# secondmind-labs/markovflow

Hardware: AMD Instinct MI355X
Metric: Kalman log-lik steps/sec (BxT) at d=6 (higher is better)
Workload: dtype f64; 1 GPU; KalmanFilter.log_likelihood B=1024/GPU T=10000 d=6 m=1 f64 (sum of two Matern-5/2, north-star target config); series_per_gpu=1024, state_dim=6, output_dim=1, parallelism=batch-sharded x1, one scalar RCCL all-reduce

## Files before the change

markovflow_amd/csrc/mf_head_carry.hpp:

```cpp
#pragma once

namespace mf {

template <int ROWB, int UNIT, typename Keep> struct HeadCarry {
    static constexpr int LINE = 128;
    static constexpr int MAXT = 2;
    static constexpr int UG = (ROWB + UNIT - 1) / UNIT;
    static constexpr int STEP = ROWB % LINE;
    static constexpr int cand(int t) {
        int n = 0;
        for (int u = 0; u < UG; ++u)
            if (Keep::keep(u, UNIT) && (u + 1) * UNIT <= LINE - 4) { if (n == t) return u; ++n; }
        return -1;
    }
    static constexpr int count_cand() { int n = 0; while (n < MAXT && cand(n) >= 0) ++n; return n; }
    static constexpr int tail_index(int u) { for (int t = 0; t < count_cand(); ++t) if (cand(t) == u) return t; return -1; }
    static constexpr unsigned carried_units(int r) {
        r &= LINE - 1;
        if (r == 0) return 0u;
        const int room = LINE - r;
        unsigned m = 0u;
        for (int u = 0; u < UG; ++u) {
            if (!Keep::keep(u, UNIT) || u * UNIT >= room) continue;
            const int t = tail_index(u);
            if (t < 0 || (u + 1) * UNIT > room) return 0u;
            m |= 1u << t;
        }
        return m;
    }
    static constexpr unsigned table(int t) {
        unsigned m = 0u;
        for (int g = 0; g < 32; ++g) if ((carried_units(4 * g) >> t) & 1u) m |= 1u << g;
        return m;
    }
    static constexpr unsigned TAB0 = table(0), TAB1 = table(1);
    static constexpr int period() { int p = 1, r = STEP; while (r % LINE) { r += STEP; ++p; } return p; }
    static constexpr int PERIOD = (ROWB % 4 == 0) ? period() : 0;
    static constexpr bool USABLE = ROWB % 4 == 0 && ROWB >= LINE && STEP != 0 && Keep::keep(UG - 1, UNIT) && (TAB0 | TAB1) != 0u;
    static constexpr int NT = USABLE ? count_cand() : 0;
    static constexpr int tail_unit(int t) { return cand(t); }

    static constexpr bool carried(unsigned addr, int t) { return (((t == 0 ? TAB0 : TAB1) >> ((addr & (LINE - 1)) >> 2)) & 1u) != 0u; }

    static constexpr unsigned consumer_bits(unsigned addr0) {
        unsigned m = 0u;
        for (int t = 0; t < NT; ++t)
            for (int p = 0; p < PERIOD; ++p) if (carried(addr0 + (unsigned)(p * STEP), t)) m |= 1u << (t * PERIOD + p);
        return m;
    }
    static constexpr unsigned producer_bits(unsigned addr0, int kind) {
        unsigned m = 0u;
        for (int p = 0; p < PERIOD; ++p) {
            bool f = true;
            if (kind >= 1 + MAXT) f = carried(addr0 + (unsigned)((p + 1) * STEP), kind - 1 - MAXT);
            else if (kind >= 1) f = !carried(addr0 + (unsigned)(p * STEP), kind - 1);
            if (f) m |= 1u << p;
        }
        return m;
    }
};

template <int ROWB, typename Keep, bool TAIL = false> struct Stream {
    static constexpr int UNIT = (ROWB >= 16) ? 16 : 4;
    static constexpr int UG = (ROWB + UNIT - 1) / UNIT;
    static constexpr int count_kept() { int n = 0; for (int u = 0; u < UG; ++u) n += Keep::keep(u, UNIT) ? 1 : 0; return n; }
    using HC = HeadCarry<ROWB, UNIT, Keep>;
    static constexpr int UB = count_kept();
    static constexpr int NT = TAIL ? HC::NT : 0;
    static constexpr int U = UB + NT;
    static constexpr int NI = U;
    static constexpr int LDS_BYTES = 64 * U * UNIT;
    static constexpr bool ALL = (UB == UG) && NT == 0;
    static constexpr int global_unit(int c) {
        int n = 0;
        for (int u = 0; u < UG; ++u) if (Keep::keep(u, UNIT)) { if (n == c) return u; ++n; }
        return -1;
    }
    static constexpr int global_offset(int c) { return c < UB ? global_unit(c) * UNIT : ROWB + HC::tail_unit(c - UB) * UNIT; }
    static constexpr int unit_kind(int c) {
        if (c >= UB) return 1 + HC::MAXT + (c - UB);
        for (int t = 0; t < NT; ++t) if (global_unit(c) == HC::tail_unit(t)) return 1 + t;
        return 0;
    }
    static constexpr int compact_unit(int gu) {
        int n = 0;
        for (int u = 0; u < gu; ++u) n += Keep::keep(u, UNIT) ? 1 : 0;
        return n;
    }
};

struct KeepAll { static constexpr bool keep(int, int) { return true; } };
template <int D, int S> struct KeepLower {
    static constexpr bool keep(int u, int unit) {
        const int lo = u * unit, hi = lo + unit;
        for (int i = 0; i < D; ++i) {
            const int a = (i * D) * S, b = (i * D + i + 1) * S;
            if (a < hi && lo < b) return true;
        }
        return false;
    }
};

}
```

markovflow_amd/csrc/mf_kf_lds.hpp:

```cpp
#pragma once
#include "mf_kernels.hpp"
#include "mf_head_carry.hpp"
#include <type_traits>
#ifndef MF_PUMPMASK
#define MF_PUMPMASK 63
#endif

namespace mf {

typedef int mf_v4i __attribute__((ext_vector_type(4)));

#define MF_POLICY_STR_0 ""
#define MF_POLICY_STR_1 " nt"
#define MF_POLICY_STR_2 " sc1"
#define MF_POLICY_STR_3 " sc0 sc1"
#define MF_POLICY_STR_4 " sc0"
#define MF_POLICY_CAT(n) MF_POLICY_STR_##n
#define MF_POLICY_OF(n) MF_POLICY_CAT(n)
#ifndef MF_POLW
#define MF_POLW 1
#endif
#ifndef MF_POLN
#define MF_POLN 0
#endif
#define MF_POLICY_WIDE MF_POLICY_OF(MF_POLW)
#define MF_POLICY_NARROW MF_POLICY_OF(MF_POLN)
#define MF_DMA_HEAD "s_nop 4\n\ts_mov_b32 %0, m0\n\ts_mov_b32 m0, %2\n\ts_nop 0\n\t"
#define MF_DMA_TAIL "s_mov_b32 m0, %0"
#define MF_DMA_X4(v, pol) "buffer_load_dwordx4 " v ", %1, 0 offen" pol " lds\n\t"
#define MF_DMA_X1(v, pol) "buffer_load_dword " v ", %1, 0 offen" pol " lds\n\t"
#define MF_DMA_STEP4 "s_add_u32 m0, m0, 0x400\n\ts_nop 0\n\t"
#define MF_DMA_STEP1 "s_add_u32 m0, m0, 0x100\n\ts_nop 0\n\t"
template <bool WIDE, int N> MF_DEV void dma_b128_group(mf_v4i srd, unsigned lds_addr, const unsigned* v) {
    unsigned keep;
    static_assert(N >= 1 && N <= 4, "group size");
#define MF_DMA_B128_BODY(POL)                                                                                                       \
    if constexpr (N == 1)                                                                                                           \
        asm volatile(MF_DMA_HEAD MF_DMA_X4("%3", POL) MF_DMA_TAIL : "=&s"(keep) : "s"(srd), "s"(lds_addr), "v"(v[0]) : "memory", "scc"); \
    else if constexpr (N == 2)                                                                                                      \
        asm volatile(MF_DMA_HEAD MF_DMA_X4("%3", POL) MF_DMA_STEP4 MF_DMA_X4("%4", POL) MF_DMA_TAIL                                 \
                     : "=&s"(keep) : "s"(srd), "s"(lds_addr), "v"(v[0]), "v"(v[1]) : "memory", "scc");                              \
    else if constexpr (N == 3)                                                                                                      \
        asm volatile(MF_DMA_HEAD MF_DMA_X4("%3", POL) MF_DMA_STEP4 MF_DMA_X4("%4", POL) MF_DMA_STEP4 MF_DMA_X4("%5", POL) MF_DMA_TAIL \
                     : "=&s"(keep) : "s"(srd), "s"(lds_addr), "v"(v[0]), "v"(v[1]), "v"(v[2]) : "memory", "scc");                   \
    else                                                                                                                            \
        asm volatile(MF_DMA_HEAD MF_DMA_X4("%3", POL) MF_DMA_STEP4 MF_DMA_X4("%4", POL) MF_DMA_STEP4 MF_DMA_X4("%5", POL)           \
                     MF_DMA_STEP4 MF_DMA_X4("%6", POL) MF_DMA_TAIL                                                                  \
                     : "=&s"(keep) : "s"(srd), "s"(lds_addr), "v"(v[0]), "v"(v[1]), "v"(v[2]), "v"(v[3]) : "memory", "scc");
    if (WIDE) { MF_DMA_B128_BODY(MF_POLICY_WIDE) } else { MF_DMA_B128_BODY(MF_POLICY_NARROW) }
#undef MF_DMA_B128_BODY
}
template <int N> MF_DEV void dma_b32_group(mf_v4i srd, unsigned lds_addr, const unsigned* v) {
    unsigned keep;
    static_assert(N >= 1 && N <= 4, "group size");
    if constexpr (N == 1)
        asm volatile(MF_DMA_HEAD MF_DMA_X1("%3", MF_POLICY_NARROW) MF_DMA_TAIL : "=&s"(keep) : "s"(srd), "s"(lds_addr), "v"(v[0]) : "memory", "scc");
    else if constexpr (N == 2)
        asm volatile(MF_DMA_HEAD MF_DMA_X1("%3", MF_POLICY_NARROW) MF_DMA_STEP1 MF_DMA_X1("%4", MF_POLICY_NARROW) MF_DMA_TAIL
                     : "=&s"(keep) : "s"(srd), "s"(lds_addr), "v"(v[0]), "v"(v[1]) : "memory", "scc");
    else if constexpr (N == 3)
        asm volatile(MF_DMA_HEAD MF_DMA_X1("%3", MF_POLICY_NARROW) MF_DMA_STEP1 MF_DMA_X1("%4", MF_POLICY_NARROW) MF_DMA_STEP1
                     MF_DMA_X1("%5", MF_POLICY_NARROW) MF_DMA_TAIL
                     : "=&s"(keep) : "s"(srd), "s"(lds_addr), "v"(v[0]), "v"(v[1]), "v"(v[2]) : "memory", "scc");
    else
        asm volatile(MF_DMA_HEAD MF_DMA_X1("%3", MF_POLICY_NARROW) MF_DMA_STEP1 MF_DMA_X1("%4", MF_POLICY_NARROW) MF_DMA_STEP1
                     MF_DMA_X1("%5", MF_POLICY_NARROW) MF_DMA_STEP1 MF_DMA_X1("%6", MF_POLICY_NARROW) MF_DMA_TAIL
                     : "=&s"(keep) : "s"(srd), "s"(lds_addr), "v"(v[0]), "v"(v[1]), "v"(v[2]), "v"(v[3]) : "memory", "scc");
}


constexpr unsigned MF_DMA_INVALID = 0xF0000000u;
constexpr unsigned long long MF_DMA_MAXREC = 0xE0000000ull;

template <typename St, typename = void> struct StreamTail { static constexpr int NT = 0, PERIOD = 1; };
template <typename St> struct StreamTail<St, std::enable_if_t<(St::NT > 0)>> { static constexpr int NT = St::NT, PERIOD = St::HC::PERIOD; };

template <typename St> struct DmaStream {
    using TL = StreamTail<St>;
    unsigned vo[St::NI];
    static constexpr int PB = TL::PERIOD;
    static constexpr int FW = TL::NT > 0 ? (St::NI * PB + 31) / 32 : 1;
    unsigned fm[FW];
    MF_DEV void init(const char* smem, int lane, int rel_tab, int gtab, unsigned base_lo = 0u) {
        const int q0 = lane / St::U, c0 = lane - q0 * St::U;
        if constexpr (TL::NT > 0) { MF_UNROLL for (int w = 0; w < FW; ++w) fm[w] = 0u; }
        MF_UNROLL for (int i = 0; i < St::NI; ++i) {
            const int a = (64 * i) / St::U, b = (64 * i) % St::U;
            int cu = c0 + b;
            const int carry = cu >= St::U ? 1 : 0;
            cu -= carry * St::U;
            const int row = q0 + a + carry;
            const unsigned rel = *reinterpret_cast<const unsigned*>(smem + rel_tab + row * 4);
            unsigned off;
            if (St::ALL) off = (unsigned)cu * St::UNIT;
            else off = *reinterpret_cast<const unsigned*>(smem + gtab + cu * 4);
            vo[i] = rel + off;
            if constexpr (TL::NT > 0) {
                static_assert(PB < 32 && 32 % PB == 0, "an instruction's schedule bits do not straddle two words");
                int kind = 0;
                MF_UNROLL for (int cc = 0; cc < St::U; ++cc) if (St::unit_kind(cc) != 0 && cu == cc) kind = St::unit_kind(cc);
                unsigned bits = (1u << PB) - 1u;
                MF_UNROLL for (int kk = 1; kk <= 2 * St::HC::MAXT; ++kk)
                    if (kind == kk) bits = St::HC::producer_bits(base_lo + rel, kk);
                fm[(i * PB) / 32] |= bits << ((i * PB) % 32);
            }
#ifdef MF_EXPERIMENT
            if (pack_base != 0xffffffffu && rel < MF_DMA_INVALID)
                vo[i] |= ((((pack_base + rel) >> 5) & 3u) << 29) | ((unsigned)(off / St::UNIT) << 24);
#endif
        }
    }
#ifdef MF_EXPERIMENT
    unsigned pack_base = 0xffffffffu;
    unsigned step_next = 0;
    bool skip_carried = false;
    MF_DEV unsigned exp_offset(unsigned v) const {
        if (pack_base == 0xffffffffu || v >= MF_DMA_INVALID) return v;
        const unsigned phase = ((v >> 29) + step_next) & 3u, gu = (v >> 24) & 31u, off = v & 0xffffffu;
        const bool carried = skip_carried && phase != 0u && gu < 8u - 2u * phase;
        return carried ? MF_DMA_INVALID : off;
    }
#endif
    template <int I0, int I1, bool SCHED = false> MF_DEV void issue(mf_v4i srd, unsigned lds_base, unsigned phase = 0u) const {
        constexpr int HI = I1 < St::NI ? I1 : St::NI;
        if constexpr (I0 < HI) {
            constexpr int N = (HI - I0) < 4 ? (HI - I0) : 4;
            unsigned voff[N];
            MF_UNROLL for (int k = 0; k < N; ++k) {
#ifdef MF_EXPERIMENT
                voff[k] = exp_offset(vo[I0 + k]);
#else
                voff[k] = vo[I0 + k];
#endif
                if constexpr (SCHED && TL::NT > 0)
                    voff[k] = ((fm[((I0 + k) * PB) / 32] >> (((I0 + k) * PB) % 32 + phase)) & 1u) ? voff[k] : MF_DMA_INVALID;
            }
            if (St::UNIT == 16) dma_b128_group<(St::UG >= 8), N>(srd, lds_base + I0 * 1024, voff);
            else dma_b32_group<N>(srd, lds_base + I0 * 256, voff);
            issue<I0 + N, I1, SCHED>(srd, lds_base, phase);
        }
    }
};

MF_DEV unsigned long long uniform64(unsigned long long x) {
    const unsigned lo = (unsigned)__builtin_amdgcn_readfirstlane((int)(unsigned)x);
    const unsigned hi = (unsigned)__builtin_amdgcn_readfirstlane((int)(unsigned)(x >> 32));
    return ((unsigned long long)hi << 32) | lo;
}

MF_DEV mf_v4i make_srd(unsigned long long base, unsigned long long end, int debug = 0) {
    unsigned long long rem = end > base ? end - base : 0ull;
    if (debug & 1) rem = 0;
    if (rem > MF_DMA_MAXREC) rem = MF_DMA_MAXREC;
    mf_v4i srd;
    srd.x = __builtin_amdgcn_readfirstlane((int)(unsigned)base);
    srd.y = __builtin_amdgcn_readfirstlane((int)((unsigned)(base >> 32) & 0xffffu));
    srd.z = __builtin_amdgcn_readfirstlane((int)(unsigned)rem);
    srd.w = 0x00020000;
    return srd;
}

template <typename T, typename St> struct RowReader {
    const char* row;
    MF_DEV RowReader(const char* smem, int lds_off, int lane) : row(smem + lds_off + lane * (St::U * St::UNIT)) {}
    MF_DEV T at(int e) const {
        const int byte = e * (int)sizeof(T);
        const int gu = byte / St::UNIT;
        const int off = St::compact_unit(gu) * St::UNIT + (byte - gu * St::UNIT);
        return *reinterpret_cast<const T*>(row + off);
    }
    MF_DEV T tail_at(int t, int k) const { return *reinterpret_cast<const T*>(row + (St::UB + t) * St::UNIT + k * (int)sizeof(T)); }
};

template <typename T, int D, int M, bool RSTEP = false, int BG = 1, bool CARRY = false> struct KfLdsCfg {
    static constexpr int S = sizeof(T);
    static constexpr int BGRP = BG;
    using StA = Stream<D * D * S, KeepAll>;
    using StC0 = Stream<D * D * S, KeepLower<D, S>>;
    using StCT = Stream<D * D * S, KeepLower<D, S>, true>;
    using Stb = Stream<BG * D * S, KeepAll>;
    using StH = Stream<BG * M * D * S, KeepAll>;
    static constexpr int YG = (M == 1) ? 4 : 1;
    using Sty = Stream<YG * M * S, KeepAll>;
    using StR = Stream<M * M * S, KeepAll>;
    static constexpr bool RS = RSTEP;
    static constexpr int QUARTER_CU = (160 * 1024) / 4;
    static constexpr int TABLE_BYTES = 5 * 256 + ((StCT::U * 4 + 15) / 16) * 16;
    static constexpr int IMAGE_T = StA::LDS_BYTES + StCT::LDS_BYTES + Stb::LDS_BYTES + StH::LDS_BYTES + ((Sty::LDS_BYTES + 15) / 16) * 16 +
                                   (RSTEP ? ((StR::LDS_BYTES + 15) / 16) * 16 : 0);
    static constexpr bool TAIL = CARRY && StCT::NT > 0 && !StC0::ALL && StCT::NI * StCT::HC::PERIOD <= 64 &&
                                 StCT::NT * StCT::HC::PERIOD <= 32 && IMAGE_T <= QUARTER_CU && TABLE_BYTES <= IMAGE_T &&
                                 (StA::NI + StCT::NI + Stb::NI + StH::NI + Sty::NI + (RSTEP ? StR::NI : 0)) < 64;
    using StC = Stream<D * D * S, KeepLower<D, S>, TAIL>;
    static constexpr int OFF_A = 0;
    static constexpr int OFF_C = OFF_A + StA::LDS_BYTES;
    static constexpr int OFF_b = OFF_C + StC::LDS_BYTES;
    static constexpr int OFF_H = OFF_b + Stb::LDS_BYTES;
    static constexpr int OFF_y = OFF_H + StH::LDS_BYTES;
    static constexpr int OFF_R = OFF_y + ((Sty::LDS_BYTES + 15) / 16) * 16;
    static constexpr int IMAGE_END = OFF_R + (RSTEP ? ((StR::LDS_BYTES + 15) / 16) * 16 : 0);
    static constexpr int OFF_relA = TAIL ? 0 : IMAGE_END;
    static constexpr int OFF_relb = OFF_relA + 256;
    static constexpr int OFF_relH = OFF_relb + 256;
    static constexpr int OFF_rely = OFF_relH + 256;
    static constexpr int OFF_relR = OFF_rely + 256;
    static constexpr int OFF_gtabC = OFF_relR + 256;
    static constexpr int LDS_TOTAL = TAIL ? IMAGE_END : OFF_gtabC + ((StC::U * 4 + 15) / 16) * 16;
    static constexpr bool SUPPORTED =
                                      (StA::NI + StC::NI + Stb::NI + StH::NI + Sty::NI + (RSTEP ? StR::NI : 0)) < 64 &&
                                      LDS_TOTAL <= 64 * 1024;
};

template <typename T, int D, int M, bool RSTEP = false> using KfChunkCfg = KfLdsCfg<T, D, M, RSTEP, 1, true>;
static_assert(KfChunkCfg<double, 6, 1>::TAIL && KfChunkCfg<double, 6, 1>::LDS_TOTAL <= 40960, "fp64 d = 6: four wavefronts per CU");

template <typename Cfg> struct KfPump {
    static constexpr int N_SMALL = Cfg::StC::NI + Cfg::Stb::NI + Cfg::StH::NI + Cfg::Sty::NI + (Cfg::RS ? Cfg::StR::NI : 0);
    static constexpr int N_BIG = Cfg::StA::NI;
    const DmaStream<typename Cfg::StA>& dA; const DmaStream<typename Cfg::StC>& dC;
    const DmaStream<typename Cfg::Stb>& db; const DmaStream<typename Cfg::StH>& dH;
    const DmaStream<typename Cfg::Sty>& dy; const DmaStream<typename Cfg::StR>& dR;
    mf_v4i sA, sC, sb, sH, sy, sR;
    unsigned lds0;
    bool more;
    bool yfetch = true;
    unsigned cphase = 0;
    template <int K> MF_DEV void small() const {
        if (!((MF_PUMPMASK >> K) & 1)) return;
        small_do<K>();
    }
    template <int K> MF_DEV void small_do() const {
        if (!more) return;
        constexpr int HC = (Cfg::StC::NI + 1) / 2;
        if (K == 0) dC.template issue<0, HC, true>(sC, lds0 + Cfg::OFF_C, cphase);
        else {
            dC.template issue<HC, 64, true>(sC, lds0 + Cfg::OFF_C, cphase);
            db.template issue<0, 64>(sb, lds0 + Cfg::OFF_b);
            dH.template issue<0, 64>(sH, lds0 + Cfg::OFF_H);
            if (yfetch) dy.template issue<0, 64>(sy, lds0 + Cfg::OFF_y);
            if (Cfg::RS) dR.template issue<0, 64>(sR, lds0 + Cfg::OFF_R);
        }
    }
    template <int K> MF_DEV void all() const {
        dC.template issue<0, 64>(sC, lds0 + Cfg::OFF_C);
        db.template issue<0, 64>(sb, lds0 + Cfg::OFF_b);
        dH.template issue<0, 64>(sH, lds0 + Cfg::OFF_H);
        dy.template issue<0, 64>(sy, lds0 + Cfg::OFF_y);
        if (Cfg::RS) dR.template issue<0, 64>(sR, lds0 + Cfg::OFF_R);
        dA.template issue<0, 64>(sA, lds0 + Cfg::OFF_A);
    }
    template <int K> MF_DEV void big() const {
        if (!((MF_PUMPMASK >> (K + 2)) & 1)) return;
        big_do<K>();
    }
    MF_DEV void unpumped() const {
        if (!((MF_PUMPMASK >> 0) & 1)) small_do<0>();
        if (!((MF_PUMPMASK >> 1) & 1)) small_do<1>();
        if (!((MF_PUMPMASK >> 2) & 1)) big_do<0>();
        if (!((MF_PUMPMASK >> 3) & 1)) big_do<1>();
        if (!((MF_PUMPMASK >> 4) & 1)) big_do<2>();
        if (!((MF_PUMPMASK >> 5) & 1)) big_do<3>();
    }
    template <int K> MF_DEV void big_do() const {
        if (!more) return;
        constexpr int Q = (Cfg::StA::NI + 3) / 4;
        dA.template issue<K * Q, (K + 1) * Q>(sA, lds0 + Cfg::OFF_A);
    }
};

template <typename T, int D, int M, bool SPIKE, bool FIRST, typename Pump>
MF_DEV void kf_lds_step(Elim<T, D, SPIKE>& E, LogAcc<T>& laC, T& acc_yry, T& acc_ww, const T (&C)[D][D],
                        const T (&mvec)[D], const T (&hk)[M * D], const T (&yk)[M], const T (&Rsh)[M * M],
                        T (&Bm)[D][D], const Pump& pump, bool active, bool sep_lane) {
    const bool sep = FIRST && sep_lane, ord = active && !sep;
    T Ci[D][D], w[D], btw[D];
    if (active) {
        tri_inv_lower<T, D>(C, Ci, laC, E.bad);
        laC.renorm();
    }
    pump.template small<0>();
    if (active) {
        trimul_lower_vec<T, D>(Ci, mvec, w);
        acc_ww += dot_self<T, D>(w);
    }
    pump.template small<1>();
    pump.template big<0>();
    if (active) {
        trimul_lower_inplace<T, D, D>(Ci, Bm);
        gemv_t<T, D, D>(Bm, w, btw);
    }
    pump.template big<1>();
    if (FIRST && active && sep) {
        syrk_tn_lower<T, D, D>(Bm, E.GU, T(1));
        MF_UNROLL for (int i = 0; i < D; ++i) E.gU[i] = -btw[i];
    }
    if (ord) {
        syrk_tn_lower<T, D, D>(Bm, E.Phi, T(1));
        MF_UNROLL for (int i = 0; i < D; ++i) E.t[i] -= btw[i];
    }
    pump.template big<2>();
    if (FIRST && active && sep) {
        neg_trimulT_lower_inplace<T, D, D>(Ci, Bm);
        MF_UNROLL for (int i = 0; i < D; ++i) MF_UNROLL for (int j = 0; j < D; ++j) E.X[i][j] = Bm[i][j];
    }
    if (ord) E.eliminate_main();
    pump.template big<3>();
    if (FIRST && active && sep) {
        trimulT_self_lower<T, D>(Ci, E.Phi);
        trimulT_lower_vec<T, D>(Ci, w, E.t);
        acc_yry += Obs<T, D, M>::apply(hk, yk, Rsh, M, E.Phi, E.t);
    }
    if (ord) {
        E.eliminate_spike();
        trsm_right_lower_t<T, D, D>(E.Phi, E.Li, Bm);
        neg_trimulT_lower_inplace<T, D, D>(Ci, Bm);
        T Dn[D][D], rn[D];
        trimulT_self_lower<T, D>(Ci, Dn);
        trimulT_lower_vec<T, D>(Ci, w, rn);
        acc_yry += Obs<T, D, M>::apply(hk, yk, Rsh, M, Dn, rn);
        E.advance(Bm, Dn, rn);
    }
}

template <typename T, int D, int M, bool SPIKE, bool RSTEP = false>
__global__ void __launch_bounds__(64) kf_chunk_lds_kernel(KfArgs<T> a, long L, RedSys<T> out) {
    using Cfg = KfChunkCfg<T, D, M, RSTEP>;
    extern __shared__ __attribute__((aligned(16))) char smem[];
    const int lane = threadIdx.x;
    const long total = a.B * a.P;
    const long id_raw = (long)blockIdx.x * 64 + lane;
    const bool valid = id_raw < total;
    const long id = valid ? id_raw : total - 1;
    const long s = id / a.P, c = id % a.P;
    const long nt = a.Tn - 1;
    const long tau0 = c * L;
    long len = nt - tau0;
    if (len > L) len = L;
    if (len < 0 || !valid) len = 0;
    constexpr int S = sizeof(T);

    const unsigned long long offA = (unsigned long long)(s * nt + tau0) * (D * D * S);
    const unsigned long long offb = (unsigned long long)(s * nt + tau0) * (D * S);
    const unsigned long long offH = (unsigned long long)(s * a.Tn + tau0 + 1) * (M * D * S);
    const unsigned long long offy = (unsigned long long)(s * a.Tn + tau0 + 1) * (M * S);
    const unsigned long long offR = (unsigned long long)(s * a.Tn + tau0 + 1) * (M * M * S);
    const unsigned long long offA0 = uniform64(offA), offb0 = uniform64(offb);
    const unsigned long long offH0 = uniform64(offH), offy0 = uniform64(offy), offR0 = uniform64(offR);
    const bool rowok = valid && len > 0;
    {
        unsigned* tab = reinterpret_cast<unsigned*>(smem);
        tab[Cfg::OFF_relA / 4 + lane] = rowok ? (unsigned)(offA - offA0) : MF_DMA_INVALID;
        tab[Cfg::OFF_relb / 4 + lane] = rowok ? (unsigned)(offb - offb0) : MF_DMA_INVALID;
        tab[Cfg::OFF_relH / 4 + lane] = rowok ? (unsigned)(offH - offH0) : MF_DMA_INVALID;
        tab[Cfg::OFF_rely / 4 + lane] = rowok ? (unsigned)(offy - offy0) : MF_DMA_INVALID;
        tab[Cfg::OFF_relR / 4 + lane] = rowok ? (unsigned)(offR - offR0) : MF_DMA_INVALID;
        if (lane < Cfg::StC::U) {
            unsigned g = 0;
            MF_UNROLL for (int cc = 0; cc < Cfg::StC::U; ++cc) if (lane == cc) g = (unsigned)Cfg::StC::global_offset(cc);
            tab[Cfg::OFF_gtabC / 4 + lane] = g;
        }
    }
    DmaStream<typename Cfg::StA> dA;
    DmaStream<typename Cfg::StC> dC;
    DmaStream<typename Cfg::Stb> db;
    DmaStream<typename Cfg::StH> dH;
    DmaStream<typename Cfg::Sty> dy;
    DmaStream<typename Cfg::StR> dR;
    unsigned long long pA = (unsigned long long)a.A + offA0, pC = (unsigned long long)a.cholQ + offA0;
    unsigned long long pb = (unsigned long long)a.b + offb0, pH = (unsigned long long)a.H + offH0;
    unsigned long long py = (unsigned long long)a.y + offy0;
    unsigned long long pR = (unsigned long long)a.Rinv + (RSTEP ? offR0 : 0ull);
    const unsigned long long eA = (unsigned long long)a.A + (unsigned long long)a.B * nt * (D * D * S);
    const unsigned long long eC = (unsigned long long)a.cholQ + (unsigned long long)a.B * nt * (D * D * S);
    const unsigned long long eb = (unsigned long long)a.b + (unsigned long long)a.B * nt * (D * S);
    const unsigned long long eH = (unsigned long long)a.H + (unsigned long long)a.B * a.Tn * (M * D * S);
    const unsigned long long ey = (unsigned long long)a.y + (unsigned long long)a.B * a.Tn * (M * S);
    const unsigned long long eR = (unsigned long long)a.Rinv + (RSTEP ? (unsigned long long)a.B * a.Tn * (M * M * S) : 0ull);
    const unsigned lds0 = (unsigned)(size_t)smem;

    Elim<T, D, SPIKE> E;
    E.init();
    LogAcc<T> laC;
    laC.init();
    T acc_yry = T(0), acc_ww = T(0);
    T Rsh[M * M];
    MF_UNROLL for (int i = 0; i < M * M; ++i) Rsh[i] = RSTEP ? (valid ? a.Rinv[(s * a.Tn) * M * M + i] : T(0)) : a.Rinv[i];
    if (valid && c == 0) {
        T C[D][D], Ci[D][D], mvec[D], w[D];
        load_lower<T, D>(a.cholP0 + s * D * D, C);
        load_vec<T, D>(a.mu0 + s * D, mvec);
        tri_inv_lower<T, D>(C, Ci, laC, E.bad);
        laC.renorm();
        trimul_lower_vec<T, D>(Ci, mvec, w);
        acc_ww += dot_self<T, D>(w);
        trimulT_self_lower<T, D>(Ci, E.Phi);
        trimulT_lower_vec<T, D>(Ci, w, E.t);
        acc_yry += Obs<T, D, M>::apply(a.H + (s * a.Tn) * M * D, a.y + (s * a.Tn) * M, Rsh, M, E.Phi, E.t);
    }

    long nsteps = len;
    MF_UNROLL for (int off = 32; off > 0; off >>= 1) {
        const long o = __shfl_xor((long long)nsteps, off);
        nsteps = o > nsteps ? o : nsteps;
    }
    nsteps = __builtin_amdgcn_readfirstlane((int)nsteps);
    asm volatile("s_waitcnt vmcnt(0) lgkmcnt(0)" ::: "memory");
#ifdef MF_EXPERIMENT
    if (a.debug & 8) {
        dA.pack_base = (unsigned)__builtin_amdgcn_readfirstlane((int)(unsigned)pA);
        dC.pack_base = (unsigned)__builtin_amdgcn_readfirstlane((int)(unsigned)pC);
    }
#endif
    dA.init(smem, lane, Cfg::OFF_relA, 0);
    dC.init(smem, lane, Cfg::OFF_relA, Cfg::OFF_gtabC, (unsigned)pC);
    db.init(smem, lane, Cfg::OFF_relb, 0);
    dH.init(smem, lane, Cfg::OFF_relH, 0);
    dy.init(smem, lane, Cfg::OFF_rely, 0);
    if (RSTEP) dR.init(smem, lane, Cfg::OFF_relR, 0);
    asm volatile("s_waitcnt lgkmcnt(0)" ::: "memory");
    using HC = typename Cfg::StC::HC;
    constexpr int NTAIL = Cfg::StC::NT, CPER = NTAIL > 0 ? HC::PERIOD : 1, UEL = Cfg::StC::UNIT / S;
    const unsigned cbits = NTAIL > 0 ? HC::consumer_bits((unsigned)((unsigned long long)a.cholQ + offA)) : 0u;
    T cv[NTAIL > 0 ? NTAIL : 1][UEL];
    MF_UNROLL for (int t = 0; t < (NTAIL > 0 ? NTAIL : 1); ++t) MF_UNROLL for (int k = 0; k < UEL; ++k) cv[t][k] = T(0);

    const RowReader<T, typename Cfg::StA> rA(smem, Cfg::OFF_A, lane);
    const RowReader<T, typename Cfg::StC> rC(smem, Cfg::OFF_C, lane);
    const RowReader<T, typename Cfg::Stb> rb(smem, Cfg::OFF_b, lane);
    const RowReader<T, typename Cfg::StH> rH(smem, Cfg::OFF_H, lane);
    const RowReader<T, typename Cfg::Sty> ry(smem, Cfg::OFF_y, lane);
    const RowReader<T, typename Cfg::StR> rR(smem, Cfg::OFF_R, lane);

    using Pump = KfPump<Cfg>;

    if (nsteps > 0) {
        Pump p0{dA, dC, db, dH, dy, dR, make_srd(pA, eA, a.debug), make_srd(pC, eC, a.debug | ((a.debug >> 2) & 1)),
                make_srd(pb, eb, a.debug | ((a.debug >> 1) & 1)), make_srd(pH, eH, a.debug | ((a.debug >> 1) & 1)),
                make_srd(py, ey, a.debug | ((a.debug >> 1) & 1)), make_srd(pR, eR, a.debug | ((a.debug >> 1) & 1)), lds0, true};
        p0.template all<0>();
    }

#ifdef MF_STAMP
#define MF_STAMP_AT(var) { unsigned long long t_; asm volatile("s_memtime %0\n\ts_waitcnt lgkmcnt(0)" : "=s"(t_) :: "memory"); var = t_; }
    unsigned long long st_wait = 0, st_io = 0, st_comp = 0, ts0 = 0, ts1 = 0, ts2 = 0, ts3 = 0;
#define MF_STAMP_ACC { asm volatile("" :: "v"(E.quad), "v"(E.Phi[0][0]) : "memory"); MF_STAMP_AT(ts3) st_wait += ts1 - ts0; st_io += ts2 - ts1; st_comp += ts3 - ts2; }
#else
#define MF_STAMP_AT(var)
#define MF_STAMP_ACC
#endif
#ifdef MF_CHECKSUM
    T cs_A = 0, cs_C = 0, cs_b = 0, cs_H = 0, cs_y = 0;
#define MF_CHECKSUM_ACC if (j < len) { MF_UNROLL for (int i = 0; i < D; ++i) { cs_b += mvec[i]; MF_UNROLL for (int jj = 0; jj < D; ++jj) { cs_A += Bm[i][jj] * T(1 + i * D + jj); if (jj <= i) cs_C += C[i][jj] * T(1 + i * D + jj); } } \
        MF_UNROLL for (int i = 0; i < M * D; ++i) cs_H += hk[i] * T(1 + i); MF_UNROLL for (int i = 0; i < M; ++i) cs_y += yk[i]; }
#else
#define MF_CHECKSUM_ACC
#endif
#ifdef MF_EXPERIMENT
#define MF_EXP_STEP_NEXT { dA.step_next = dC.step_next = (unsigned)(j + 1); dA.skip_carried = dC.skip_carried = (a.debug & 8) != 0; }
#else
#define MF_EXP_STEP_NEXT
#endif
#define MF_NOPUMP_ISSUE pump.unpumped();
#define MF_KF_LDS_STEP(FIRST)                                                                                         \
    {                                                                                                                 \
        MF_STAMP_AT(ts0)                                                                                              \
        asm volatile("s_waitcnt vmcnt(0)" ::: "memory");                                                              \
        MF_STAMP_AT(ts1)                                                                                              \
        const bool more = (j + 1 < nsteps);                                                                           \
        const bool yfetch = ((j + 1) % Cfg::YG) == 0;                                                                 \
        pA += D * D * S; pC += D * D * S; pb += D * S; pH += M * D * S; if (RSTEP) pR += M * M * S;                   \
        if (yfetch) py += Cfg::YG * M * S;                                                                            \
        T C[D][D], mvec[D], hk[M * D], yk[M];                                                                         \
        MF_UNROLL for (int i = 0; i < D; ++i) MF_UNROLL for (int jj = 0; jj <= i; ++jj) C[i][jj] = rC.at(i * D + jj); \
        if constexpr (NTAIL > 0) {                                                                                    \
               \
               \
            MF_UNROLL for (int t = 0; t < NTAIL; ++t) {                                                               \
                const bool got = !(FIRST) && ((cbits >> (t * CPER + (int)(j & (CPER - 1)))) & 1u) != 0u;              \
                MF_UNROLL for (int i = 0; i < D; ++i) MF_UNROLL for (int jj = 0; jj <= i; ++jj)                       \
                    if (((i * D + jj) * S) / Cfg::StC::UNIT == HC::tail_unit(t))                                      \
                        C[i][jj] = got ? cv[t][(i * D + jj) - HC::tail_unit(t) * UEL] : C[i][jj];                     \
                MF_UNROLL for (int k = 0; k < UEL; ++k) cv[t][k] = rC.tail_at(t, k);                                  \
            }                                                                                                         \
        }                                                                                                             \
        MF_UNROLL for (int i = 0; i < D; ++i) mvec[i] = rb.at(i);                                                     \
        MF_UNROLL for (int i = 0; i < M * D; ++i) hk[i] = rH.at(i);                                                   \
        MF_UNROLL for (int i = 0; i < M; ++i)                                                                         \
            yk[i] = *reinterpret_cast<const T*>(ry.row + ((int)(j % Cfg::YG) * M + i) * (int)sizeof(T));              \
        if (RSTEP) { MF_UNROLL for (int i = 0; i < M * M; ++i) Rsh[i] = rR.at(i); }                                    \
        T Bm[D][D];                                                                                                   \
        MF_UNROLL for (int i = 0; i < D; ++i) MF_UNROLL for (int jj = 0; jj < D; ++jj) Bm[i][jj] = rA.at(i * D + jj); \
        asm volatile("s_waitcnt lgkmcnt(0)" ::: "memory");                                                            \
        MF_CHECKSUM_ACC                                                                                               \
        MF_STAMP_AT(ts2)                                                                                              \
        const Pump pump{dA, dC, db, dH, dy, dR, make_srd(pA, eA, a.debug),                                            \
                        make_srd(pC, eC, a.debug | ((a.debug >> 2) & 1)),                                             \
                        make_srd(pb, eb, a.debug | ((a.debug >> 1) & 1)),                                             \
                        make_srd(pH, eH, a.debug | ((a.debug >> 1) & 1)),                                             \
                        make_srd(py, ey, a.debug | ((a.debug >> 1) & 1)),                                             \
                        make_srd(pR, eR, a.debug | ((a.debug >> 1) & 1)), lds0, more, yfetch,                         \
                        (unsigned)((j + 1) & (CPER - 1))};                                                            \
        MF_EXP_STEP_NEXT                                                                                              \
        MF_NOPUMP_ISSUE                                                                                               \
        const bool active = j < len;                                                                                  \
        kf_lds_step<T, D, M, SPIKE, FIRST>(E, laC, acc_yry, acc_ww, C, mvec, hk, yk, Rsh, Bm, pump, active, c > 0);    \
        if (E.bad && first_bad < 0) first_bad = tau0 + j;                                                             \
        MF_STAMP_ACC                                                                                                  \
    }
    long j = 0;
    long first_bad = -1;
    if (nsteps > 0) MF_KF_LDS_STEP(true)
    for (j = 1; j < nsteps; ++j) MF_KF_LDS_STEP(false)
#undef MF_KF_LDS_STEP
    asm volatile("s_waitcnt vmcnt(0)" ::: "memory");
    if (valid) {
        const T scalar = T(-0.5) * (acc_yry + acc_ww) + T(0.5) * E.quad - laC.value() - E.laL.value();
        store_chunk<T, D, SPIKE>(out, id, E, scalar);
        if (E.bad && a.info) raise_pivot(a.info, s * a.Tn + (first_bad < 0 ? tau0 : first_bad));
#ifdef MF_CHECKSUM
        out.GU[id * D * D + 0] = cs_A; out.GU[id * D * D + 1] = cs_C; out.GU[id * D * D + 2] = cs_b;
        out.gU[id * D + 0] = cs_H; out.gU[id * D + 1] = cs_y;
#endif
#ifdef MF_STAMP
        if (lane == 0) {
            out.GU[id * D * D + 0] = (T)st_wait; out.GU[id * D * D + 1] = (T)st_io; out.GU[id * D * D + 2] = (T)st_comp;
        }
#endif
    }
}

}
```

Measured before the change: 7.782 billion steps/s.

## Generalize head-carry tail units to the A stream and more tail slots

Generalizes the head-carry scheme (reusing cache-line tail units fetched with the previous row instead of re-fetching them) to support up to 8 tail units and to apply it to the transition matrix A stream as well as the Cholesky Q stream. The configuration now picks the largest workable tail count per stream at compile time. The static asserts indicate that for fp64 d=6, C keeps 2 tails and A gets none, so the benchmarked path is essentially unchanged. The fp32 path gains tailing on both wide streams, at the cost of extra register state and selection logic.

```diff
diff --git a/markovflow_amd/csrc/mf_head_carry.hpp b/markovflow_amd/csrc/mf_head_carry.hpp
--- a/markovflow_amd/csrc/mf_head_carry.hpp
+++ b/markovflow_amd/csrc/mf_head_carry.hpp
@@ -1,10 +1,12 @@
 #pragma once
+#include <type_traits>
 
 namespace mf {
 
-template <int ROWB, int UNIT, typename Keep> struct HeadCarry {
+template <int ROWB, int UNIT, typename Keep, int MAXT_ = 2> struct HeadCarry {
     static constexpr int LINE = 128;
-    static constexpr int MAXT = 2;
+    static constexpr int MAXT = MAXT_;
+    static_assert(MAXT >= 1 && MAXT <= 8, "tail units: one bit each in carried_units, LINE / UNIT at the most");
     static constexpr int UG = (ROWB + UNIT - 1) / UNIT;
     static constexpr int STEP = ROWB % LINE;
     static constexpr int cand(int t) {
@@ -14,7 +16,8 @@
         return -1;
     }
     static constexpr int count_cand() { int n = 0; while (n < MAXT && cand(n) >= 0) ++n; return n; }
-    static constexpr int tail_index(int u) { for (int t = 0; t < count_cand(); ++t) if (cand(t) == u) return t; return -1; }
+    static constexpr int NC = count_cand();
+    static constexpr int tail_index(int u) { for (int t = 0; t < NC; ++t) if (cand(t) == u) return t; return -1; }
     static constexpr unsigned carried_units(int r) {
         r &= LINE - 1;
         if (r == 0) return 0u;
@@ -33,19 +36,27 @@
         for (int g = 0; g < 32; ++g) if ((carried_units(4 * g) >> t) & 1u) m |= 1u << g;
         return m;
     }
-    static constexpr unsigned TAB0 = table(0), TAB1 = table(1);
+    template <int K = 0> static constexpr unsigned tab(int t) {
+        if constexpr (K >= MAXT) return 0u;
+        else { constexpr unsigned v = table(K); return t == K ? v : tab<K + 1>(t); }
+    }
+    static constexpr unsigned any_table() { unsigned m = 0u; for (int g = 0; g < 32; ++g) m |= carried_units(4 * g); return m; }
     static constexpr int period() { int p = 1, r = STEP; while (r % LINE) { r += STEP; ++p; } return p; }
     static constexpr int PERIOD = (ROWB % 4 == 0) ? period() : 0;
-    static constexpr bool USABLE = ROWB % 4 == 0 && ROWB >= LINE && STEP != 0 && Keep::keep(UG - 1, UNIT) && (TAB0 | TAB1) != 0u;
-    static constexpr int NT = USABLE ? count_cand() : 0;
+    static constexpr bool USABLE = ROWB % 4 == 0 && ROWB >= LINE && STEP != 0 && Keep::keep(UG - 1, UNIT) && any_table() != 0u;
+    static constexpr int NT = USABLE ? NC : 0;
     static constexpr int tail_unit(int t) { return cand(t); }
+    static constexpr int carrying_phases() { int n = 0; for (int p = 0; p < PERIOD; ++p) n += carried_units(p * STEP) != 0u ? 1 : 0; return n; }
 
-    static constexpr bool carried(unsigned addr, int t) { return (((t == 0 ? TAB0 : TAB1) >> ((addr & (LINE - 1)) >> 2)) & 1u) != 0u; }
+    static constexpr bool carried(unsigned addr, int t) { return ((tab(t) >> ((addr & (LINE - 1)) >> 2)) & 1u) != 0u; }
 
-    static constexpr unsigned consumer_bits(unsigned addr0) {
-        unsigned m = 0u;
+    static constexpr int SCHED_BITS = NT * (PERIOD > 0 ? PERIOD : 1);
+    using sched_t = std::conditional_t<(SCHED_BITS > 32), unsigned long long, unsigned>;
+    static constexpr sched_t consumer_bits(unsigned addr0) {
+        static_assert(SCHED_BITS <= 64, "consumer schedule: at most two registers");
+        sched_t m = 0u;
         for (int t = 0; t < NT; ++t)
-            for (int p = 0; p < PERIOD; ++p) if (carried(addr0 + (unsigned)(p * STEP), t)) m |= 1u << (t * PERIOD + p);
+            for (int p = 0; p < PERIOD; ++p) if (carried(addr0 + (unsigned)(p * STEP), t)) m |= (sched_t)1u << (t * PERIOD + p);
         return m;
     }
     static constexpr unsigned producer_bits(unsigned addr0, int kind) {
@@ -58,25 +69,35 @@
         }
         return m;
     }
+    static constexpr unsigned producer_bits_any(unsigned addr0, int kind) {
+        const bool tail = kind >= 1 + MAXT;
+        const unsigned tb = tab(tail ? kind - 1 - MAXT : kind - 1);
+        const unsigned a = addr0 + (tail ? (unsigned)STEP : 0u);
+        unsigned m = 0u;
+        for (int p = 0; p < PERIOD; ++p) if ((tb >> (((a + (unsigned)(p * STEP)) & (LINE - 1)) >> 2)) & 1u) m |= 1u << p;
+        const unsigned all = PERIOD >= 32 ? ~0u : (1u << (PERIOD & 31)) - 1u;
+        return kind < 1 ? all : (tail ? m : all & ~m);
+    }
 };
 
-template <int ROWB, typename Keep, bool TAIL = false> struct Stream {
+template <int ROWB, typename Keep, bool TAIL = false, int MAXT_ = 2> struct Stream {
     static constexpr int UNIT = (ROWB >= 16) ? 16 : 4;
     static constexpr int UG = (ROWB + UNIT - 1) / UNIT;
     static constexpr int count_kept() { int n = 0; for (int u = 0; u < UG; ++u) n += Keep::keep(u, UNIT) ? 1 : 0; return n; }
-    using HC = HeadCarry<ROWB, UNIT, Keep>;
+    using HC = HeadCarry<ROWB, UNIT, Keep, MAXT_>;
     static constexpr int UB = count_kept();
     static constexpr int NT = TAIL ? HC::NT : 0;
     static constexpr int U = UB + NT;
     static constexpr int NI = U;
     static constexpr int LDS_BYTES = 64 * U * UNIT;
-    static constexpr bool ALL = (UB == UG) && NT == 0;
     static constexpr int global_unit(int c) {
         int n = 0;
         for (int u = 0; u < UG; ++u) if (Keep::keep(u, UNIT)) { if (n == c) return u; ++n; }
         return -1;
     }
     static constexpr int global_offset(int c) { return c < UB ? global_unit(c) * UNIT : ROWB + HC::tail_unit(c - UB) * UNIT; }
+    static constexpr bool linear() { for (int c = 0; c < U; ++c) if (global_offset(c) != c * UNIT) return false; return true; }
+    static constexpr bool ALL = (UB == UG) && (NT == 0 || linear());
     static constexpr int unit_kind(int c) {
         if (c >= UB) return 1 + HC::MAXT + (c - UB);
         for (int t = 0; t < NT; ++t) if (global_unit(c) == HC::tail_unit(t)) return 1 + t;
diff --git a/markovflow_amd/csrc/mf_kf_lds.hpp b/markovflow_amd/csrc/mf_kf_lds.hpp
--- a/markovflow_amd/csrc/mf_kf_lds.hpp
+++ b/markovflow_amd/csrc/mf_kf_lds.hpp
@@ -100,8 +100,10 @@
                 int kind = 0;
                 MF_UNROLL for (int cc = 0; cc < St::U; ++cc) if (St::unit_kind(cc) != 0 && cu == cc) kind = St::unit_kind(cc);
                 unsigned bits = (1u << PB) - 1u;
-                MF_UNROLL for (int kk = 1; kk <= 2 * St::HC::MAXT; ++kk)
-                    if (kind == kk) bits = St::HC::producer_bits(base_lo + rel, kk);
+                if constexpr (St::HC::MAXT <= 2) {
+                    MF_UNROLL for (int kk = 1; kk <= 2 * St::HC::MAXT; ++kk)
+                        if (kind == kk) bits = St::HC::producer_bits(base_lo + rel, kk);
+                } else bits = St::HC::producer_bits_any(base_lo + rel, kind);
                 fm[(i * PB) / 32] |= bits << ((i * PB) % 32);
             }
 #ifdef MF_EXPERIMENT
@@ -172,26 +174,22 @@
     MF_DEV T tail_at(int t, int k) const { return *reinterpret_cast<const T*>(row + (St::UB + t) * St::UNIT + k * (int)sizeof(T)); }
 };
 
-template <typename T, int D, int M, bool RSTEP = false, int BG = 1, bool CARRY = false> struct KfLdsCfg {
+#ifndef MF_KF_MAXTAIL_A
+#define MF_KF_MAXTAIL_A 7
+#endif
+template <typename T, int D, int M, bool RSTEP, int BG, int WA, int WC> struct KfLdsLayout {
     static constexpr int S = sizeof(T);
     static constexpr int BGRP = BG;
-    using StA = Stream<D * D * S, KeepAll>;
-    using StC0 = Stream<D * D * S, KeepLower<D, S>>;
-    using StCT = Stream<D * D * S, KeepLower<D, S>, true>;
+    using StA = Stream<D * D * S, KeepAll, (WA > 0), (WA > 0 ? WA : 2)>;
+    using StC = Stream<D * D * S, KeepLower<D, S>, (WC > 0), (WC > 0 ? WC : 2)>;
     using Stb = Stream<BG * D * S, KeepAll>;
     using StH = Stream<BG * M * D * S, KeepAll>;
     static constexpr int YG = (M == 1) ? 4 : 1;
     using Sty = Stream<YG * M * S, KeepAll>;
     using StR = Stream<M * M * S, KeepAll>;
     static constexpr bool RS = RSTEP;
+    static constexpr bool TAIL = WA > 0 || WC > 0;
     static constexpr int QUARTER_CU = (160 * 1024) / 4;
-    static constexpr int TABLE_BYTES = 5 * 256 + ((StCT::U * 4 + 15) / 16) * 16;
-    static constexpr int IMAGE_T = StA::LDS_BYTES + StCT::LDS_BYTES + Stb::LDS_BYTES + StH::LDS_BYTES + ((Sty::LDS_BYTES + 15) / 16) * 16 +
-                                   (RSTEP ? ((StR::LDS_BYTES + 15) / 16) * 16 : 0);
-    static constexpr bool TAIL = CARRY && StCT::NT > 0 && !StC0::ALL && StCT::NI * StCT::HC::PERIOD <= 64 &&
-                                 StCT::NT * StCT::HC::PERIOD <= 32 && IMAGE_T <= QUARTER_CU && TABLE_BYTES <= IMAGE_T &&
-                                 (StA::NI + StCT::NI + Stb::NI + StH::NI + Sty::NI + (RSTEP ? StR::NI : 0)) < 64;
-    using StC = Stream<D * D * S, KeepLower<D, S>, TAIL>;
     static constexpr int OFF_A = 0;
     static constexpr int OFF_C = OFF_A + StA::LDS_BYTES;
     static constexpr int OFF_b = OFF_C + StC::LDS_BYTES;
@@ -199,20 +197,48 @@
     static constexpr int OFF_y = OFF_H + StH::LDS_BYTES;
     static constexpr int OFF_R = OFF_y + ((Sty::LDS_BYTES + 15) / 16) * 16;
     static constexpr int IMAGE_END = OFF_R + (RSTEP ? ((StR::LDS_BYTES + 15) / 16) * 16 : 0);
-    static constexpr int OFF_relA = TAIL ? 0 : IMAGE_END;
+    static constexpr int TABLE_BYTES = 5 * 256 + ((StC::U * 4 + 15) / 16) * 16;
+    static constexpr bool OVER = TAIL && IMAGE_END + TABLE_BYTES > QUARTER_CU;
+    static constexpr int OFF_relA = OVER ? 0 : IMAGE_END;
     static constexpr int OFF_relb = OFF_relA + 256;
     static constexpr int OFF_relH = OFF_relb + 256;
     static constexpr int OFF_rely = OFF_relH + 256;
     static constexpr int OFF_relR = OFF_rely + 256;
     static constexpr int OFF_gtabC = OFF_relR + 256;
-    static constexpr int LDS_TOTAL = TAIL ? IMAGE_END : OFF_gtabC + ((StC::U * 4 + 15) / 16) * 16;
-    static constexpr bool SUPPORTED =
-                                      (StA::NI + StC::NI + Stb::NI + StH::NI + Sty::NI + (RSTEP ? StR::NI : 0)) < 64 &&
-                                      LDS_TOTAL <= 64 * 1024;
+    static constexpr int LDS_TOTAL = OVER ? IMAGE_END : OFF_gtabC + ((StC::U * 4 + 15) / 16) * 16;
+    static constexpr int N_DMA = StA::NI + StC::NI + Stb::NI + StH::NI + Sty::NI + (RSTEP ? StR::NI : 0);
+    template <typename St, int W> static constexpr bool stream_ok() {
+        if constexpr (W == 0) return true;
+        else return St::NT == W && (D * D * S) % St::UNIT == 0 && St::HC::PERIOD < 32 && 32 % St::HC::PERIOD == 0 && W * St::HC::PERIOD <= 64 &&
+                    2 * St::HC::carrying_phases() >= St::HC::PERIOD;
+    }
+    static constexpr bool TAIL_OK = stream_ok<StA, WA>() && stream_ok<StC, WC>() && StA::ALL &&
+                                    (!TAIL || (LDS_TOTAL <= QUARTER_CU && (!OVER || TABLE_BYTES <= IMAGE_END) && N_DMA < 64));
+    static constexpr bool SUPPORTED = N_DMA < 64 && LDS_TOTAL <= 64 * 1024;
 };
+template <typename T, int D, int M, bool RSTEP, int BG, int W = 7> constexpr int kf_pick_tail_c() {
+    if constexpr (W == 0) return 0;
+    else if constexpr (KfLdsLayout<T, D, M, RSTEP, BG, 0, W>::TAIL_OK) return W;
+    else return kf_pick_tail_c<T, D, M, RSTEP, BG, W - 1>();
+}
+template <typename T, int D, int M, bool RSTEP, int BG, int WC, int W = MF_KF_MAXTAIL_A> constexpr int kf_pick_tail_a() {
+    if constexpr (W == 0 || WC == 0) return 0;
+    else if constexpr (KfLdsLayout<T, D, M, RSTEP, BG, W, WC>::TAIL_OK) return W;
+    else return kf_pick_tail_a<T, D, M, RSTEP, BG, WC, W - 1>();
+}
+template <typename T, int D, int M, bool RSTEP, int BG, bool CARRY> struct KfTailPick {
+    static constexpr int WC = CARRY ? kf_pick_tail_c<T, D, M, RSTEP, BG>() : 0;
+    static constexpr int WA = CARRY ? kf_pick_tail_a<T, D, M, RSTEP, BG, WC>() : 0;
+};
+template <typename T, int D, int M, bool RSTEP = false, int BG = 1, bool CARRY = false>
+struct KfLdsCfg : KfLdsLayout<T, D, M, RSTEP, BG, KfTailPick<T, D, M, RSTEP, BG, CARRY>::WA, KfTailPick<T, D, M, RSTEP, BG, CARRY>::WC> {};
 
 template <typename T, int D, int M, bool RSTEP = false> using KfChunkCfg = KfLdsCfg<T, D, M, RSTEP, 1, true>;
-static_assert(KfChunkCfg<double, 6, 1>::TAIL && KfChunkCfg<double, 6, 1>::LDS_TOTAL <= 40960, "fp64 d = 6: four wavefronts per CU");
+static_assert(KfChunkCfg<double, 6, 1>::StC::NT == 2 && KfChunkCfg<double, 6, 1>::StA::NT == 0 && KfChunkCfg<double, 6, 1>::OVER &&
+              KfChunkCfg<double, 6, 1>::LDS_TOTAL == 40960, "fp64 d = 6: chol Q's units {0, 3}, four wavefronts per CU");
+static_assert(KfChunkCfg<float, 6, 1>::StC::NT == 6 && KfChunkCfg<float, 6, 1>::StA::NT == MF_KF_MAXTAIL_A && !KfChunkCfg<float, 6, 1>::OVER &&
+              KfChunkCfg<float, 6, 1>::LDS_TOTAL <= 40960 && KfChunkCfg<float, 6, 1>::N_DMA <= 35,
+              "fp32 d = 6: both wide streams tailed, four wavefronts per CU");
 
 template <typename Cfg> struct KfPump {
     static constexpr int N_SMALL = Cfg::StC::NI + Cfg::Stb::NI + Cfg::StH::NI + Cfg::Sty::NI + (Cfg::RS ? Cfg::StR::NI : 0);
@@ -225,6 +251,7 @@
     bool more;
     bool yfetch = true;
     unsigned cphase = 0;
+    unsigned aphase = 0;
     template <int K> MF_DEV void small() const {
         if (!((MF_PUMPMASK >> K) & 1)) return;
         small_do<K>();
@@ -264,7 +291,7 @@
     template <int K> MF_DEV void big_do() const {
         if (!more) return;
         constexpr int Q = (Cfg::StA::NI + 3) / 4;
-        dA.template issue<K * Q, (K + 1) * Q>(sA, lds0 + Cfg::OFF_A);
+        dA.template issue<K * Q, (K + 1) * Q, true>(sA, lds0 + Cfg::OFF_A, aphase);
     }
 };
 
@@ -411,7 +438,7 @@
         dC.pack_base = (unsigned)__builtin_amdgcn_readfirstlane((int)(unsigned)pC);
     }
 #endif
-    dA.init(smem, lane, Cfg::OFF_relA, 0);
+    dA.init(smem, lane, Cfg::OFF_relA, 0, (unsigned)pA);
     dC.init(smem, lane, Cfg::OFF_relA, Cfg::OFF_gtabC, (unsigned)pC);
     db.init(smem, lane, Cfg::OFF_relb, 0);
     dH.init(smem, lane, Cfg::OFF_relH, 0);
@@ -420,9 +447,14 @@
     asm volatile("s_waitcnt lgkmcnt(0)" ::: "memory");
     using HC = typename Cfg::StC::HC;
     constexpr int NTAIL = Cfg::StC::NT, CPER = NTAIL > 0 ? HC::PERIOD : 1, UEL = Cfg::StC::UNIT / S;
-    const unsigned cbits = NTAIL > 0 ? HC::consumer_bits((unsigned)((unsigned long long)a.cholQ + offA)) : 0u;
+    const typename HC::sched_t cbits = NTAIL > 0 ? HC::consumer_bits((unsigned)((unsigned long long)a.cholQ + offA)) : 0u;
     T cv[NTAIL > 0 ? NTAIL : 1][UEL];
     MF_UNROLL for (int t = 0; t < (NTAIL > 0 ? NTAIL : 1); ++t) MF_UNROLL for (int k = 0; k < UEL; ++k) cv[t][k] = T(0);
+    using HCA = typename Cfg::StA::HC;
+    constexpr int NTA = Cfg::StA::NT, APER = NTA > 0 ? HCA::PERIOD : 1, UELA = Cfg::StA::UNIT / S;
+    const typename HCA::sched_t abits = NTA > 0 ? HCA::consumer_bits((unsigned)((unsigned long long)a.A + offA)) : 0u;
+    T av[NTA > 0 ? NTA : 1][UELA];
+    MF_UNROLL for (int t = 0; t < (NTA > 0 ? NTA : 1); ++t) MF_UNROLL for (int k = 0; k < UELA; ++k) av[t][k] = T(0);
 
     const RowReader<T, typename Cfg::StA> rA(smem, Cfg::OFF_A, lane);
     const RowReader<T, typename Cfg::StC> rC(smem, Cfg::OFF_C, lane);
@@ -490,6 +522,15 @@
         if (RSTEP) { MF_UNROLL for (int i = 0; i < M * M; ++i) Rsh[i] = rR.at(i); }                                    \
         T Bm[D][D];                                                                                                   \
         MF_UNROLL for (int i = 0; i < D; ++i) MF_UNROLL for (int jj = 0; jj < D; ++jj) Bm[i][jj] = rA.at(i * D + jj); \
+        if constexpr (NTA > 0) {                                                                                      \
+            MF_UNROLL for (int t = 0; t < NTA; ++t) {                                                                 \
+                const bool got = !(FIRST) && ((abits >> (t * APER + (int)(j & (APER - 1)))) & 1u) != 0u;              \
+                MF_UNROLL for (int i = 0; i < D; ++i) MF_UNROLL for (int jj = 0; jj < D; ++jj)                        \
+                    if (((i * D + jj) * S) / Cfg::StA::UNIT == HCA::tail_unit(t))                                     \
+                        Bm[i][jj] = got ? av[t][(i * D + jj) - HCA::tail_unit(t) * UELA] : Bm[i][jj];                 \
+                MF_UNROLL for (int k = 0; k < UELA; ++k) av[t][k] = rA.tail_at(t, k);                                 \
+            }                                                                                                         \
+        }                                                                                                             \
         asm volatile("s_waitcnt lgkmcnt(0)" ::: "memory");                                                            \
         MF_CHECKSUM_ACC                                                                                               \
         MF_STAMP_AT(ts2)                                                                                              \
@@ -499,7 +540,7 @@
                         make_srd(pH, eH, a.debug | ((a.debug >> 1) & 1)),                                             \
                         make_srd(py, ey, a.debug | ((a.debug >> 1) & 1)),                                             \
                         make_srd(pR, eR, a.debug | ((a.debug >> 1) & 1)), lds0, more, yfetch,                         \
-                        (unsigned)((j + 1) & (CPER - 1))};                                                            \
+                        (unsigned)((j + 1) & (CPER - 1)), (unsigned)((j + 1) & (APER - 1))};                          \
         MF_EXP_STEP_NEXT                                                                                              \
         MF_NOPUMP_ISSUE                                                                                               \
         const bool active = j < len;                                                                                  \
```

Result: no change. 7.781 billion steps/s (median of 2 runs) (-0.0%).
